# zzyunzhi/object-intrinsics

Hardware: AMD Instinct MI355X
Metric: rendered rays/sec (64x64 img, 128 samples/ray) + D-images/sec (higher is better)
Workload: dtype f32 via f16x3 (fp32 operands split into 2 fp16 limbs = 22 mantissa bits, 3 fp16 MFMAs per product, fp32 accumulate: 2^-22 relative per product, 1e-4 parity path); 1 GPU; C2: 1x64x64 crop per GPU, 64+64 samples/ray, 1 up-sampling step(s), Generator.forward (render + Phong maps) + ADADiscriminatorView forward; parallelism=dp1 (independent renders, no data-path collective)

## Files before the change

### object-intrinsics_amd/build.py

```python
import hashlib
import os
import subprocess
import sys

HERE = os.path.dirname(os.path.abspath(__file__))
CSRC = os.path.join(HERE, "csrc")
OUT_DIR = os.path.join(HERE, "oi_amd")
LIB = os.path.join(OUT_DIR, "liboi_hip.so")
STAMP = os.path.join(OUT_DIR, ".liboi_hip.stamp")
SOURCES = ["mlp.hip", "mlp_fwd3.hip", "mlp_fwd3b.hip", "color_head.hip", "render.hip", "disc.hip", "disc_small.hip", "disc_large.hip", "mlp_bwd.hip", "render_bwd.hip", "disc_bwd.hip", "optim.hip", "loss.hip", "mesh.hip", "relight.hip"]
FLAGS = ["--offload-arch=gfx950", "-O3", "-std=c++17", "-fPIC", "-Wno-unused-value"] + os.environ.get("OI_FLAGS", "").split()
EXTRA = {"mlp_fwd3.hip": ["-mllvm", "-amdgpu-mfma-vgpr-form=1"],
         "mlp_fwd3b.hip": ["-mllvm", "-amdgpu-mfma-vgpr-form=1", "-fno-slp-vectorize"],
         "mlp_bwd.hip": ["-mllvm", "-amdgpu-mfma-vgpr-form=1"]}


def _hipcc():
    for c in (os.environ.get("HIPCC"), "/opt/rocm/bin/hipcc", "hipcc"):
        if c and (os.path.isabs(c) and os.path.exists(c) or not os.path.isabs(c)):
            return c
    raise RuntimeError("hipcc not found")


def _sources():
    return [s for s in SOURCES if os.path.exists(os.path.join(CSRC, s))]


def _digest():
    h = hashlib.sha256()
    files = [os.path.join(CSRC, f) for f in sorted(os.listdir(CSRC))]
    inc = os.path.join(os.path.dirname(HERE), "include")
    files += [os.path.join(inc, f) for f in sorted(os.listdir(inc))]
    for f in files:
        with open(f, "rb") as fh:
            h.update(os.path.basename(f).encode())
            h.update(fh.read())
    h.update(" ".join(FLAGS).encode())
    h.update(repr(EXTRA).encode())
    return h.hexdigest()


def build(force=False, verbose=True):
    dig = _digest()
    if not force and os.path.exists(LIB) and os.path.exists(STAMP) and open(STAMP).read() == dig:
        return LIB
    hipcc = _hipcc()
    objs = []
    procs = []
    os.makedirs(os.path.join(HERE, "build"), exist_ok=True)
    for s in _sources():
        o = os.path.join(HERE, "build", s.replace(".hip", ".o"))
        cmd = [hipcc, *FLAGS, *EXTRA.get(s, []), "-c", os.path.join(CSRC, s), "-o", o]
        if verbose:
            print(" ".join(cmd), flush=True)
        procs.append((s, subprocess.Popen(cmd, stdout=subprocess.PIPE, stderr=subprocess.STDOUT)))
        objs.append(o)
    for s, p in procs:
        out, _ = p.communicate()
        if p.returncode != 0:
            raise RuntimeError(f"hipcc failed on {s}:\n{out.decode()}")
    cmd = [hipcc, "--offload-arch=gfx950", "-shared", "-fPIC", "-o", LIB, *objs]
    if verbose:
        print(" ".join(cmd), flush=True)
    subprocess.check_call(cmd)
    with open(STAMP, "w") as fh:
        fh.write(dig)
    return LIB


if __name__ == "__main__":
    print(build(force="--force" in sys.argv))
```

### object-intrinsics_amd/csrc/mlp.hip

```cpp
#include <cstdlib>

#include <algorithm>

#include "mlp_common.h"
#include "f3_blob.h"

namespace {

using namespace oimlp;

__global__ void film_params_kernel(const float* __restrict__ style_w, const float* __restrict__ style_b,
                                   const float* __restrict__ z, float* __restrict__ w_out,
                                   const float* __restrict__ gw, const float* __restrict__ gb,
                                   const float* __restrict__ bw, const float* __restrict__ bb,
                                   float* __restrict__ gamma, float* __restrict__ beta, int NL) {
  __shared__ float h[2][64];
  const int e = blockIdx.x, t = threadIdx.x;
  if (z != nullptr) {
    if (t < 64) h[0][t] = z[e * 64 + t];
    __syncthreads();
    int cur = 0;
    for (int l = 0; l < 3; ++l) {
      if (t < 64) {
        const float* wr = style_w + (l * 64 + t) * 64;
// ... 119 lines not shown
    __syncthreads();
    for (int o = part; o < 64; o += 4) atomicAdd(d_style_w + (l * 64 + o) * 64 + t, dh[cur][o] * h[l][t]);
    if (tid < 64) {
      float acc = 0.f;
#pragma unroll 8
      for (int o = 0; o < 64; ++o) acc = fmaf(dh[cur][o], W[l][o][t], acc);
      dh[cur ^ 1][t] = acc;
    }
    __syncthreads();
    cur ^= 1;
  }
  if (d_z != nullptr && tid < 64) d_z[e * 64 + t] = dh[cur][t];
}

__device__ __forceinline__ float mat_elem(const float* wh, const float* wv, int m, int row, int k) {
  if (m < 7) return wh[((size_t)m * C + row) * C + k];
  if (m < 14) return wh[((size_t)(m - 7) * C + k) * C + row];
  if (m == 14) return wv[(size_t)row * (C + 3) + k];
  return wv[(size_t)k * (C + 3) + row];
}

template <int PREC>
__device__ float image_scale(const float* wh, const float* wv, int m, float* red, float* inv, float* bad,
                             float* rowsum = nullptr) {
  *bad = 0.f;
  if (PREC != OI_PREC_F16X3) {
    *inv = 1.f;
    return 1.f;
  }
  float mx = 0.f;
  for (int i = threadIdx.x; i < C * C; i += 256) {
    const float a = fabsf(mat_elem(wh, wv, m, i >> 7, i & 127));
    mx = a <= 3.0e38f ? fmaxf(mx, a) : __builtin_inff();
    if (rowsum != nullptr) atomicAdd(rowsum + (i >> 7), a);
  }
  red[threadIdx.x] = mx;
  __syncthreads();
  for (int o = 128; o > 0; o >>= 1) {
    if ((int)threadIdx.x < o) red[threadIdx.x] = fmaxf(red[threadIdx.x], red[threadIdx.x + o]);
    __syncthreads();
  }
  mx = red[0];
  __syncthreads();
  *bad = mx <= 3.0e38f ? 0.f : 1.f;
  int eb = (__builtin_bit_cast(int, mx) >> 23) & 0xff;
  eb = eb < 14 ? 14 : (eb > 254 ? 254 : eb);
  *inv = __builtin_bit_cast(float, (eb - 13) << 23);
  return __builtin_bit_cast(float, (267 - eb) << 23);
}

constexpr int PK_PER = 8;

template <int PREC>
__global__ void pack_weights_kernel(const float* __restrict__ w0, const float* __restrict__ b0,
                                    const float* __restrict__ wh, const float* __restrict__ bh,
                                    const float* __restrict__ wsig, const float* __restrict__ bsig,
                                    const float* __restrict__ wv, const float* __restrict__ bv,
                                    const float* __restrict__ wrgb, const float* __restrict__ brgb,
                                    char* __restrict__ packed) {
  float* hdr = reinterpret_cast<float*>(packed);
  __shared__ float red[256];
  if (blockIdx.y == NMAT) {
   for (int idx = blockIdx.x * blockDim.x + threadIdx.x; idx < H_FLOATS; idx += gridDim.x * blockDim.x) {
    if ((idx >= H_WSCALE && idx < H_WSCALE + NMAT) || (idx >= H_BOUND && idx < H_BOUND + NMAT) ||
        (idx >= H_STATUS && idx < H_STATUS + NMAT))
      continue;
    float v = 0.f;
    if (idx < H_SIG) {
      int f = idx >> 2, j = idx & 3;
      v = j < 3 ? w0[f * 3 + j] : 0.f;
    } else if (idx < H_TABV) {
      int i = idx - H_SIG;
      v = i < C ? wsig[i] : (i == C ? bsig[0] : 0.f);
    } else if (idx < H_RGB) {
      int i = idx - H_TABV, f = i >> 2, j = i & 3;
      v = j < 3 ? wv[(size_t)f * (C + 3) + C + j] : 0.f;
    } else if (idx < H_TABS_END) {
      int i = idx - H_RGB;
      v = i < 3 * C ? wrgb[i] : (i < 3 * C + 3 ? brgb[i - 3 * C] : 0.f);
    } else if (idx < H_BIAS + 9 * C) {
      int i = idx - H_BIAS, l = i / C, f = i % C;
      v = l == 0 ? b0[f] : (l < 8 ? bh[(l - 1) * C + f] : bv[f]);
    }
    hdr[idx] = v;
   }
    return;
  }
  const int m = blockIdx.y;
  float inv, bad;
  __shared__ float rowsum[C];
  if (threadIdx.x < C) rowsum[threadIdx.x] = 0.f;
  __syncthreads();
  const float wscale = image_scale<PREC>(wh, wv, m, red, &inv, &bad, blockIdx.x == 0 ? rowsum : nullptr);
  if (blockIdx.x == 0 && threadIdx.x == 0) {
    hdr[H_WSCALE + m] = inv;
    hdr[H_STATUS + m] = bad;
  }
  if (blockIdx.x == 0) {
    float rs = 0.f;
    if (threadIdx.x < C) {
      if (PREC == OI_PREC_F16X3) rs = rowsum[threadIdx.x];
      else for (int k = 0; k < C; ++k) rs += fabsf(mat_elem(wh, wv, m, threadIdx.x, k));
    }
    red[threadIdx.x] = rs;
    __syncthreads();
    for (int o = 128; o > 0; o >>= 1) {
      if ((int)threadIdx.x < o) red[threadIdx.x] = fmaxf(red[threadIdx.x], red[threadIdx.x + o]);
      __syncthreads();
    }
    if (threadIdx.x == 0) hdr[H_BOUND + m] = red[0] * wscale;
    __syncthreads();
  }
  for (int part = 0; part < PK_PER; ++part) {
  const int idx = (blockIdx.x * PK_PER + part) * blockDim.x + threadIdx.x;
  if (idx >= C * C) return;
  if (m < 7 || m == 14)
    reinterpret_cast<float*>(packed + plain_off(PREC))[(size_t)(m < 7 ? m : 7) * C * C + idx] =
        mat_elem(wh, wv, m, idx >> 7, idx & 127);
  char* base = packed + H_BYTES + (size_t)m * layer_bytes(PREC);
  if (PREC == OI_PREC_F32) {
    const int k = idx & 3, lane = (idx >> 2) & 63, g = (idx >> 8) & 15, t = idx >> 12;
    const int q = 4 * g + k, h = lane >> 5, i = lane & 31;
    reinterpret_cast<float*>(base)[idx] = mat_elem(wh, wv, m, 32 * t + i, feat_of(q, h));
  } else {
    const int ip = idx & 7, lane = (idx >> 3) & 63, s = (idx >> 9) & 7, t = idx >> 12;
    const int q = 8 * s + ip, h = lane >> 5, i = lane & 31;
    const float v = mat_elem(wh, wv, m, 32 * t + i, feat_of(q, h)) * wscale;
    if (PREC == OI_PREC_F16X3) {
      const _Float16 fh = (_Float16)v;
      reinterpret_cast<_Float16*>(base)[idx] = fh;
      reinterpret_cast<_Float16*>(base + 32768)[idx] = (_Float16)(v - (float)fh);
      continue;
    }
    const __bf16 hi = (__bf16)v;
    reinterpret_cast<__bf16*>(base)[idx] = hi;
    if (PREC == OI_PREC_BF16X3) reinterpret_cast<__bf16*>(base + 32768)[idx] = (__bf16)(v - (float)hi);
    if (PREC == OI_PREC_BF16X6) {
      const float r1 = v - (float)hi;
      const __bf16 mid = (__bf16)r1;
      reinterpret_cast<__bf16*>(base + 32768)[idx] = mid;
      reinterpret_cast<__bf16*>(base + 65536)[idx] = (__bf16)(r1 - (float)mid);
    }
  }
  }
}


template <bool FAST>
__device__ __forceinline__ float sin_rev(float phi_rev) {
  return __builtin_amdgcn_sinf(FAST ? phi_rev : __builtin_amdgcn_fractf(phi_rev));
}
template <bool FAST, bool FULL, int SRC, class SCR, bool REV = false>
__device__ __forceinline__ void film_sin2(const char* lds, const LaneOff& o, const LayOff& y, const f32x16 (&acc)[4],
                                          float (&act)[64], const SCR& ws, int slot, int tab_imm, float vx,
                                          float vy, float vz) {
#pragma unroll
  for (int g = 0; g < 16; ++g) {
    const int t = g >> 2, rr = g & 3;
    const f32x4 gm = lds_f4(lds, grp_f0(g) * 4, y.f16);
    const f32x4 bt = lds_f4(lds, (C + grp_f0(g)) * 4, y.f16);
    f32x4 cv;
#pragma unroll
    for (int k = 0; k < 4; ++k) {
      float u;
      if constexpr (SRC == 0) {
        u = acc[t][4 * rr + k];
      } else {
        const f32x4 w = lds_f4(lds, V2_TABS + tab_imm * 4 + (grp_f0(g) + k) * 16, o.h64);
        const float d = fmaf(vz, w[2], fmaf(vy, w[1], vx * w[0]));
        u = SRC == 1 ? d : acc[t][4 * rr + k] + d;
      }
      const float phi = fmaf(gm[k], u, bt[k]);
      if constexpr (REV) {
        act[4 * g + k] = sin_rev<FAST>(phi);
      } else {
        float s, c;
        sincos_<FAST>(phi, s, c);
        act[4 * g + k] = s;
        cv[k] = gm[k] * c;
      }
    }
    if constexpr (FULL) ws.store(slot, g, o, cv);
    if ((g & 1) == 1) __builtin_amdgcn_sched_barrier(0);
  }
}

template <bool FAST, bool FULL, bool REV, class SCR>
__device__ __forceinline__ void layer_fwd_pipelined(const char* lds, const LaneOff& o, const LayOff& y,
                                                    f32x16 (&acc)[4], float (&act)[64], const SCR& ws, int slot) {
  f16x8 bh[8], bl[8];
#pragma unroll
  for (int s = 0; s < 8; ++s) split8_pairs(&act[8 * s], bh[s], bl[s]);
  f32x4 gm, bt, cv;
  auto film_val = [&](int tb, int s, int j) {
    const int g = tb * 4 + (s >> 1), k = 2 * (s & 1) + j;
    if (k == 0) {
      gm = lds_f4(lds, grp_f0(g) * 4, y.f16);
      bt = lds_f4(lds, (C + grp_f0(g)) * 4, y.f16);
    }
    const float phi = fmaf(gm[k], acc[tb][2 * s + j], bt[k]);
    if constexpr (REV) {
      act[4 * g + k] = sin_rev<FAST>(phi);
    } else {
      float sn, cs;
      sincos_<FAST>(phi, sn, cs);
      act[4 * g + k] = sn;
      cv[k] = gm[k] * cs;
    }
    if constexpr (FULL) {
      if (k == 3) ws.store(slot, g, o, cv);
    }
  };
  auto film_part = [&](int tb, int s) {
    film_val(tb, s, 0);
    film_val(tb, s, 1);
  };
  f32x4 ah = lds_f4(lds, 0, y.wl), al = lds_f4(lds, 0, y.wh), ahn = ah, aln = al;
#pragma unroll
  for (int t = 0; t < 4; ++t) {
#pragma unroll
    for (int r = 0; r < 16; ++r) acc[t][r] = 0.f;
#pragma unroll
    for (int s = 0; s < 8; ++s) {
      const int nxt = t * 8 + s + 1;
      if (nxt < 32) {
        ahn = lds_f4(lds, nxt * 1024, y.wl);
        aln = lds_f4(lds, nxt * 1024, y.wh);
      }
      const f16x8 wh = __builtin_bit_cast(f16x8, ah);
      const f16x8 wl = __builtin_bit_cast(f16x8, al);
      acc[t] = __builtin_amdgcn_mfma_f32_32x32x16_f16(wl, bh[s], acc[t], 0, 0, 0);
      if (t > 0) {
        film_val(t - 1, s, 0);
        __builtin_amdgcn_sched_barrier(0);
      }
      acc[t] = __builtin_amdgcn_mfma_f32_32x32x16_f16(wh, bl[s], acc[t], 0, 0, 0);
      if (t > 0) {
        film_val(t - 1, s, 1);
        __builtin_amdgcn_sched_barrier(0);
      }
      acc[t] = __builtin_amdgcn_mfma_f32_32x32x16_f16(wh, bh[s], acc[t], 0, 0, 0);
      __builtin_amdgcn_sched_barrier(0);
      ah = ahn;
      al = aln;
    }
  }
#pragma unroll
  for (int s = 0; s < 8; ++s) {
    film_part(3, s);
    if (s & 1) __builtin_amdgcn_sched_barrier(0);
  }
}

__device__ __forceinline__ void zero_acc(f32x16 (&acc)[4]) {
#pragma unroll
  for (int t = 0; t < 4; ++t)
#pragma unroll
    for (int r = 0; r < 16; ++r) acc[t][r] = 0.f;
}

#ifdef OI_PROF
__device__ unsigned long long oi_prof[16];
#define PROF_T(i)                                                  \
  do {                                                             \
    const unsigned long long t_ = __builtin_readcyclecounter();    \
    pacc[i] += t_ - tprev;                                         \
    tprev = t_;                                                    \
  } while (0)
#else
#define PROF_T(i)
#endif

#define OI_SDF_LATTICE 0
#include "sdf_mlp_kernel.inc"
#undef OI_SDF_LATTICE

#define OI_LATTICE_POINT(x, y, z)                                                                            \
  do {                                                                                                       \
    const unsigned loc_ = (unsigned)(pt - (long long)e * n_per_elem), nyz_ = (unsigned)lat_ny * lat_nz;      \
    const unsigned ix_ = loc_ / nyz_, r_ = loc_ - ix_ * nyz_, iy_ = r_ / (unsigned)lat_nz;                   \
    x = xs[ix_], y = ys[iy_], z = zs[r_ - iy_ * (unsigned)lat_nz];                                           \
  } while (0)
#define OI_SDF_LATTICE 1
#include "sdf_mlp_kernel.inc"
#undef OI_SDF_LATTICE
#undef OI_LATTICE_POINT

template <int PREC, bool FAST, bool FULL>
int launch_mlp_variant(const float* pts, const char* pk, const float* gamma, const float* beta, float* sdf, float* grad,
                       float* rgb, float* feat, char* scratch, int B, long long n, hipStream_t st) {
  constexpr int NWV = V2_WAVES;
  constexpr int LDS_BYTES = v2_lds_total(PREC);
  static const int per_dev = [] {
    const char* v = getenv("OI_V2_PERSIST");
    if (v && v[0] == '0') return 0;
    int dev = 0, cus = 256;
    (void)hipGetDevice(&dev);
    (void)hipDeviceGetAttribute(&cus, hipDeviceAttributeMultiprocessorCount, dev);
    return cus > 0 ? cus : 256;
  }();
  const int tiles = oi::cdiv(n, NWV * WAVE_PTS);
  const bool persist = !FULL && v2_two_slots(PREC) && per_dev > 0;
  dim3 grid(persist ? std::min(tiles, std::max(1, per_dev / B)) : tiles, B), block(64 * NWV);
  auto k = sdf_mlp_kernel<PREC, FAST, FULL>;
  (void)hipFuncSetAttribute(reinterpret_cast<const void*>(k), hipFuncAttributeMaxDynamicSharedMemorySize, LDS_BYTES);
  hipLaunchKernelGGL(k, grid, block, LDS_BYTES, st, pts, pk, gamma, beta, sdf, grad, rgb, feat, scratch, n);
  return oi::check_launch("oi_sdf_mlp_fwd");
}

template <int PREC, bool FAST>
int launch_lattice(const float* xs, const float* ys, const float* zs, int ny, int nz, float scale, const char* pk,
                   const float* gamma, const float* beta, float* out, int B, long long n, hipStream_t st) {
  constexpr int NWV = V2_WAVES;
  constexpr int LDS_BYTES = v2_lds_total(PREC);
  static const int cus = [] {
    int dev = 0, c = 256;
    (void)hipGetDevice(&dev);
    (void)hipDeviceGetAttribute(&c, hipDeviceAttributeMultiprocessorCount, dev);
    return c > 0 ? c : 256;
  }();
  const int tiles = oi::cdiv(n, NWV * WAVE_PTS);
  dim3 grid(v2_two_slots(PREC) ? std::min(tiles, std::max(1, cus / B)) : tiles, B), block(64 * NWV);
  auto k = sdf_lattice_kernel<PREC, FAST, false>;
  static std::atomic<unsigned long long> set{0};
  int dev = 0;
  (void)hipGetDevice(&dev);
  if (dev >= 64 || !((set.load() >> dev) & 1ull)) {
    if (hipFuncSetAttribute(reinterpret_cast<const void*>(k), hipFuncAttributeMaxDynamicSharedMemorySize, LDS_BYTES) !=
        hipSuccess)
      return oi::fail(OI_ERR_LAUNCH, "oi_sdf_lattice: hipFuncSetAttribute(%d B of LDS) failed", LDS_BYTES);
    if (dev < 64) set.fetch_or(1ull << dev);
  }
  hipLaunchKernelGGL(k, grid, block, LDS_BYTES, st, xs, ys, zs, ny, nz, scale, pk, gamma, beta, out, n);
  return oi::check_launch("oi_sdf_lattice");
}

template <int PREC, bool FAST>
int launch_mlp(const float* pts, const void* packed, const float* gamma, const float* beta, float* sdf,
               float* grad, float* rgb, float* feat, void* scratch, int B, long long n, hipStream_t st) {
  const char* pk = reinterpret_cast<const char*>(packed);
  if (grad != nullptr) {
    if constexpr (PREC == OI_PREC_F16X3 || PREC == OI_PREC_BF16)
      return oi::fail(OI_ERR_INVALID_ARG, "oi_sdf_mlp_fwd: precision %d with the gradient has no v2 kernel", PREC);
    else
      return launch_mlp_variant<PREC, FAST, true>(pts, pk, gamma, beta, sdf, grad, rgb, feat,
                                                  reinterpret_cast<char*>(scratch), B, n, st);
  }
  return launch_mlp_variant<PREC, FAST, false>(pts, pk, gamma, beta, sdf, nullptr, nullptr, feat, nullptr, B, n, st);
}

template <bool FAST>
__global__ void selftest_sincos_kernel(const float* __restrict__ x, float* __restrict__ s, float* __restrict__ c,
                                       long long n) {
  const long long i = (long long)blockIdx.x * blockDim.x + threadIdx.x;
  if (i >= n) return;
  float sv, cv;
  sincos_<FAST>(x[i], sv, cv);
  s[i] = sv;
  c[i] = cv;
}

}

extern "C" {

int oi_film_params(const float* style_w, const float* style_b, const float* z, float* w_out, const float* gw,
                   const float* gb, const float* bw, const float* bb, float* gamma, float* beta, int B, int NL,
                   oi_stream_t stream) {
  OI_REQUIRE(B > 0 && NL >= 0, "oi_film_params: B=%d NL=%d", B, NL);
  OI_REQUIRE(w_out && (NL == 0 || (gw && gb && bw && bb && gamma && beta)), "oi_film_params: null pointer");
  OI_REQUIRE(z == nullptr || (style_w && style_b), "oi_film_params: z given without style weights");
  hipLaunchKernelGGL(film_params_kernel, dim3(B, NL > 0 ? NL : 1), dim3(C), 0, oi::as_stream(stream), style_w, style_b, z, w_out,
                     gw, gb, bw, bb, gamma, beta, NL);
  return oi::check_launch("oi_film_params");
}

#ifdef OI_PROF
int oi_prof_read(unsigned long long* out, int reset) {
  (void)hipDeviceSynchronize();
  (void)hipMemcpyFromSymbol(out, HIP_SYMBOL(oi_prof), sizeof(unsigned long long) * 16);
  if (reset) {
    unsigned long long z[16] = {0};
    (void)hipMemcpyToSymbol(HIP_SYMBOL(oi_prof), z, sizeof(z));
  }
  return 0;
}
#endif

int oi_film_params_bwd(const float* d_gamma, const float* d_beta, const float* w, const float* gw, const float* bw,
                       float* d_gw, float* d_gb, float* d_bw, float* d_bb, float* d_w, const float* style_w,
                       const float* style_b, const float* z, float* d_style_w, float* d_style_b, float* d_z, int B,
                       int NL, oi_stream_t stream) {
  OI_REQUIRE(B > 0 && NL >= 0 && (NL > 0 || z != nullptr), "oi_film_params_bwd: B=%d NL=%d", B, NL);
  OI_REQUIRE(d_w && (NL == 0 || (d_gamma && d_beta && w && gw && bw && d_gw && d_gb && d_bw && d_bb)),
             "oi_film_params_bwd: null pointer");
  OI_REQUIRE(z == nullptr || (style_w && style_b && d_style_w && d_style_b),
             "oi_film_params_bwd: style backward needs style_w, style_b, d_style_w, d_style_b");
  hipStream_t st = oi::as_stream(stream);
  int rc = OI_OK;
  if (NL > 0) {
    hipLaunchKernelGGL(film_heads_bwd_kernel, dim3(NL), dim3(256), 0, st, d_gamma, d_beta, w, gw, bw, d_gw, d_gb, d_bw,
                       d_bb, d_w, B, NL);
    rc = oi::check_launch("oi_film_params_bwd(heads)");
  }
  if (rc != OI_OK || z == nullptr) return rc;
  hipLaunchKernelGGL(style_bwd_kernel, dim3(B), dim3(256), 0, st, style_w, style_b, z, d_w, d_style_w, d_style_b, d_z);
  return oi::check_launch("oi_film_params_bwd(style)");
}

size_t oi_mlp_packed_bytes(int prec) { return packed_total_bytes(prec); }

int oi_mlp_pack_weights(const float* w0, const float* b0, const float* wh, const float* bh, const float* wsig,
                        const float* bsig, const float* wv, const float* bv, const float* wrgb, const float* brgb,
                        void* packed, int prec, oi_stream_t stream) {
  OI_REQUIRE(w0 && b0 && wh && bh && wsig && bsig && wv && bv && wrgb && brgb && packed,
             "oi_mlp_pack_weights: null pointer");
  dim3 grid(C * C / (256 * PK_PER), NMAT + 1), block(256);
  char* p = reinterpret_cast<char*>(packed);
  hipStream_t st = oi::as_stream(stream);
  switch (prec) {
    case OI_PREC_F32:
      hipLaunchKernelGGL(pack_weights_kernel<OI_PREC_F32>, grid, block, 0, st, w0, b0, wh, bh, wsig, bsig, wv, bv,
                         wrgb, brgb, p);
      break;
    case OI_PREC_BF16X3:
      hipLaunchKernelGGL(pack_weights_kernel<OI_PREC_BF16X3>, grid, block, 0, st, w0, b0, wh, bh, wsig, bsig, wv, bv,
                         wrgb, brgb, p);
      break;
    case OI_PREC_BF16:
      hipLaunchKernelGGL(pack_weights_kernel<OI_PREC_BF16>, grid, block, 0, st, w0, b0, wh, bh, wsig, bsig, wv, bv,
                         wrgb, brgb, p);
      break;
    case OI_PREC_BF16X6:
      hipLaunchKernelGGL(pack_weights_kernel<OI_PREC_BF16X6>, grid, block, 0, st, w0, b0, wh, bh, wsig, bsig, wv, bv,
                         wrgb, brgb, p);
      break;
    case OI_PREC_F16X3:
      hipLaunchKernelGGL(pack_weights_kernel<OI_PREC_F16X3>, grid, block, 0, st, w0, b0, wh, bh, wsig, bsig, wv, bv,
                         wrgb, brgb, p);
      break;
    default:
      return oi::fail(OI_ERR_INVALID_ARG, "oi_mlp_pack_weights: bad precision %d", prec);
  }
  return oi::check_launch("oi_mlp_pack_weights");
}

int oi_selftest_sincos(const float* x, float* s, float* c, long long n, int fast, oi_stream_t stream) {
  OI_REQUIRE(x && s && c && n > 0, "oi_selftest_sincos: bad argument");
  if (fast)
    hipLaunchKernelGGL(selftest_sincos_kernel<true>, dim3(oi::cdiv(n, 256)), dim3(256), 0, oi::as_stream(stream), x, s, c, n);
  else
    hipLaunchKernelGGL(selftest_sincos_kernel<false>, dim3(oi::cdiv(n, 256)), dim3(256), 0, oi::as_stream(stream), x, s, c, n);
  return oi::check_launch("oi_selftest_sincos");
}

int oi_mlp_pack_status(const void* packed, oi_stream_t stream) {
  OI_REQUIRE(packed, "oi_mlp_pack_status: null pointer");
  hipStream_t st = oi::as_stream(stream);
  static thread_local float host[H_FLOATS];
  if (hipMemcpyAsync(host, packed, sizeof(host), hipMemcpyDeviceToHost, st) != hipSuccess || hipStreamSynchronize(st) != hipSuccess)
    return oi::fail(OI_ERR_LAUNCH, "oi_mlp_pack_status: reading the packed header failed");
  for (int m = 0; m < NMAT; ++m)
    if (host[H_STATUS + m] != 0.f)
      return oi::fail(OI_ERR_UNSUPPORTED, "oi_mlp_pack_status: weight image %d holds a non-finite value (inf / NaN)", m);
  for (int i = 0; i < H_BIAS + 9 * C; ++i)
    if (!(host[i] >= -3.0e38f && host[i] <= 3.0e38f))
      return oi::fail(OI_ERR_UNSUPPORTED, "oi_mlp_pack_status: non-finite first-layer / head weight or bias (header float %d)", i);
  return OI_OK;
}

size_t oi_mlp_scratch_bytes(int B, long long n_per_elem) {
  const long long tiles = (n_per_elem + V2_TILE - 1) / V2_TILE;
  return (size_t)B * tiles * V2_WAVES * NSLOT * 16 * 64 * 16;
}

size_t oi_mlp_scratch_bytes_prec(int B, long long n_per_elem, int prec) {
  if (prec == OI_PREC_F16X3) return oimlp::full3_scratch_bytes(B, n_per_elem);
  if (prec == OI_PREC_BF16) return oimlp::full3_bf16_scratch_bytes(B);
  return oi_mlp_scratch_bytes(B, n_per_elem);
}

int oi_sdf_mlp_fwd(const float* pts, const void* packed, const float* gamma, const float* beta, float* sdf,
                   float* grad, float* rgb, float* feat, void* scratch, int B, long long n_per_elem, int prec,
                   int fast_trig, oi_stream_t stream) {
  return oi_sdf_mlp_fwd_ex(pts, packed, gamma, beta, sdf, grad, rgb, feat, scratch, B, n_per_elem, prec, fast_trig, 0, stream);
}

size_t oi_mlp_f3_blob_offset(int B, long long n_per_elem) { return oimlp::full3_blob_offset(B, n_per_elem); }
size_t oi_mlp_f3_blob_bytes(void) { return (size_t)oif3::F3_BLOB; }

int oi_sdf_mlp_fwd_ex(const float* pts, const void* packed, const float* gamma, const float* beta, float* sdf,
                      float* grad, float* rgb, float* feat, void* scratch, int B, long long n_per_elem, int prec,
                      int fast_trig, int flags, oi_stream_t stream) {
  OI_REQUIRE(pts && packed && gamma && beta && sdf, "oi_sdf_mlp_fwd: null pointer");
  OI_REQUIRE((flags & ~OI_MLP_BLOB_READY) == 0, "oi_sdf_mlp_fwd_ex: unknown flag bits %d", flags);
  OI_REQUIRE(!(flags & OI_MLP_BLOB_READY) || (prec == OI_PREC_F16X3 && grad != nullptr),
             "oi_sdf_mlp_fwd_ex: OI_MLP_BLOB_READY applies to the OI_PREC_F16X3 pass with the gradient");
  OI_REQUIRE(B > 0 && n_per_elem > 0, "oi_sdf_mlp_fwd: B=%d n=%lld", B, n_per_elem);
  OI_REQUIRE(grad != nullptr || rgb == nullptr, "oi_sdf_mlp_fwd: rgb requires grad");
  OI_REQUIRE(grad == nullptr || scratch != nullptr, "oi_sdf_mlp_fwd: grad requires scratch");
  hipStream_t st = oi::as_stream(stream);
  if (prec == OI_PREC_F16X3 && grad != nullptr)
    return oimlp::launch_full3_f16x3(pts, packed, gamma, beta, sdf, grad, rgb, feat, scratch, B, n_per_elem, fast_trig,
                                     (flags & OI_MLP_BLOB_READY) != 0, st);
  if (prec == OI_PREC_BF16 && grad != nullptr)
    return oimlp::launch_full3_bf16(pts, packed, gamma, beta, sdf, grad, rgb, feat, scratch, B, n_per_elem, fast_trig, st);
#define OI_MLP_CASE(P)                                                                                        \
  case P:                                                                                                     \
    return fast_trig ? launch_mlp<P, true>(pts, packed, gamma, beta, sdf, grad, rgb, feat, scratch, B, n_per_elem, st) \
                     : launch_mlp<P, false>(pts, packed, gamma, beta, sdf, grad, rgb, feat, scratch, B, n_per_elem, st);
  switch (prec) {
    OI_MLP_CASE(OI_PREC_F32)
    OI_MLP_CASE(OI_PREC_BF16X3)
    OI_MLP_CASE(OI_PREC_BF16)
    OI_MLP_CASE(OI_PREC_BF16X6)
    OI_MLP_CASE(OI_PREC_F16X3)
    default:
      return oi::fail(OI_ERR_INVALID_ARG, "oi_sdf_mlp_fwd: bad precision %d", prec);
  }
#undef OI_MLP_CASE
}

int oi_sdf_lattice(const void* packed, const float* gamma, const float* beta, int B, const float* xs, const float* ys,
                   const float* zs, int nx, int ny, int nz, float scale, float* out, int prec, int fast_trig,
                   oi_stream_t stream) {
  OI_REQUIRE(packed && gamma && beta && xs && ys && zs && out, "oi_sdf_lattice: null pointer");
  OI_REQUIRE(B > 0 && nx > 0 && ny > 0 && nz > 0, "oi_sdf_lattice: B=%d nx=%d ny=%d nz=%d", B, nx, ny, nz);
  const long long n = (long long)nx * ny * nz;
  OI_REQUIRE(n < (1ll << 31), "oi_sdf_lattice: %d x %d x %d = %lld points per element (at most 2^31 - 1)", nx, ny, nz, n);
  const char* pk = reinterpret_cast<const char*>(packed);
  hipStream_t st = oi::as_stream(stream);
#define OI_LAT_CASE(P)                                                                                           \
  case P:                                                                                                        \
    return fast_trig ? launch_lattice<P, true>(xs, ys, zs, ny, nz, scale, pk, gamma, beta, out, B, n, st)        \
                     : launch_lattice<P, false>(xs, ys, zs, ny, nz, scale, pk, gamma, beta, out, B, n, st);
  switch (prec) {
    OI_LAT_CASE(OI_PREC_F32)
    OI_LAT_CASE(OI_PREC_BF16X3)
    OI_LAT_CASE(OI_PREC_BF16)
    OI_LAT_CASE(OI_PREC_BF16X6)
    OI_LAT_CASE(OI_PREC_F16X3)
    default:
      return oi::fail(OI_ERR_INVALID_ARG, "oi_sdf_lattice: bad precision %d", prec);
  }
#undef OI_LAT_CASE
}

}
```

### object-intrinsics_amd/csrc/mlp_common.h

```cpp
#pragma once
#include "oi_common.h"

namespace oimlp {

typedef float f32x16 __attribute__((ext_vector_type(16)));
typedef float f32x4 __attribute__((ext_vector_type(4)));
typedef __bf16 bf16x8 __attribute__((ext_vector_type(8)));
typedef _Float16 f16x8 __attribute__((ext_vector_type(8)));

constexpr int C = 128;
constexpr int NL_SDF = 8;
constexpr int NMAT = 16;
constexpr int TILE_PTS = 128;
constexpr int WAVE_PTS = 32;
constexpr int NSLOT = 9;

constexpr int H_TAB0 = 0;
constexpr int H_SIG = 512;
constexpr int H_TABV = 656;
constexpr int H_RGB = 1168;
constexpr int H_TABS_END = 1568;
constexpr int H_BIAS = 1568;
constexpr int H_WSCALE = 2720;
constexpr int H_BOUND = 2736;
// ... 123 lines not shown
        for (int t = 0; t < 4; ++t)
          acc[t] = __builtin_amdgcn_mfma_f32_32x32x2f32(a[t][k], act[4 * g + k], acc[t], 0, 0, 0);
      }
      if (g & 1) hook(g >> 1);
      __builtin_amdgcn_sched_barrier(0);
#pragma unroll
      for (int t = 0; t < 4; ++t) a[t] = an[t];
    }
  } else if constexpr (PREC == OI_PREC_BF16X6) {
#pragma unroll
    for (int s = 0; s < 8; ++s) {
      bf16x8 bh, bm, bl;
#pragma unroll
      for (int i = 0; i < 8; ++i) {
        const float v = act[8 * s + i];
        bh[i] = (__bf16)v;
        const float r1 = v - (float)bh[i];
        bm[i] = (__bf16)r1;
        bl[i] = (__bf16)(r1 - (float)bm[i]);
      }
#pragma unroll
      for (int t = 0; t < 4; ++t) {
        const bf16x8 wh = __builtin_bit_cast(bf16x8, lds_f4(lds, (t * 8 + s) * 1024, y.wl));
        const bf16x8 wm = __builtin_bit_cast(bf16x8, lds_f4(lds, (t * 8 + s) * 1024, y.wh));
        const bf16x8 wl = __builtin_bit_cast(bf16x8, lds_f4(lds, (t * 8 + s) * 1024, y.wq));
        acc[t] = __builtin_amdgcn_mfma_f32_32x32x16_bf16(wl, bh, acc[t], 0, 0, 0);
        acc[t] = __builtin_amdgcn_mfma_f32_32x32x16_bf16(wh, bl, acc[t], 0, 0, 0);
        acc[t] = __builtin_amdgcn_mfma_f32_32x32x16_bf16(wm, bm, acc[t], 0, 0, 0);
        acc[t] = __builtin_amdgcn_mfma_f32_32x32x16_bf16(wm, bh, acc[t], 0, 0, 0);
        acc[t] = __builtin_amdgcn_mfma_f32_32x32x16_bf16(wh, bm, acc[t], 0, 0, 0);
        acc[t] = __builtin_amdgcn_mfma_f32_32x32x16_bf16(wh, bh, acc[t], 0, 0, 0);
      }
      hook(s);
      __builtin_amdgcn_sched_barrier(0);
    }
  } else if constexpr (PREC == OI_PREC_F16X3) {
    f32x4 ah[4], ahn[4], al[4], aln[4];
#pragma unroll
    for (int t = 0; t < 4; ++t) {
      ah[t] = lds_f4(lds, (t * 8 + 0) * 1024, y.wl);
      al[t] = lds_f4(lds, (t * 8 + 0) * 1024, y.wh);
    }
#pragma unroll
    for (int s = 0; s < 8; ++s) {
      if (s < 7) {
#pragma unroll
        for (int t = 0; t < 4; ++t) {
          ahn[t] = lds_f4(lds, (t * 8 + s + 1) * 1024, y.wl);
          aln[t] = lds_f4(lds, (t * 8 + s + 1) * 1024, y.wh);
        }
      }
      f16x8 bh, bl;
      split8_pairs(&act[8 * s], bh, bl);
#pragma unroll
      for (int t = 0; t < 4; ++t) {
        const f16x8 wh = __builtin_bit_cast(f16x8, ah[t]);
        const f16x8 wl = __builtin_bit_cast(f16x8, al[t]);
        acc[t] = __builtin_amdgcn_mfma_f32_32x32x16_f16(wl, bh, acc[t], 0, 0, 0);
        acc[t] = __builtin_amdgcn_mfma_f32_32x32x16_f16(wh, bl, acc[t], 0, 0, 0);
        acc[t] = __builtin_amdgcn_mfma_f32_32x32x16_f16(wh, bh, acc[t], 0, 0, 0);
      }
      hook(s);
      __builtin_amdgcn_sched_barrier(0);
#pragma unroll
      for (int t = 0; t < 4; ++t) {
        ah[t] = ahn[t];
        al[t] = aln[t];
      }
    }
  } else {
    f32x4 ah[4], ahn[4], al[4], aln[4];
#pragma unroll
    for (int t = 0; t < 4; ++t) {
      ah[t] = lds_f4(lds, (t * 8 + 0) * 1024, y.wl);
      if constexpr (PREC == OI_PREC_BF16X3) al[t] = lds_f4(lds, (t * 8 + 0) * 1024, y.wh);
    }
#pragma unroll
    for (int s = 0; s < 8; ++s) {
      if (s < 7) {
#pragma unroll
        for (int t = 0; t < 4; ++t) {
          ahn[t] = lds_f4(lds, (t * 8 + s + 1) * 1024, y.wl);
          if constexpr (PREC == OI_PREC_BF16X3) aln[t] = lds_f4(lds, (t * 8 + s + 1) * 1024, y.wh);
        }
      }
      bf16x8 bh, bl;
#pragma unroll
      for (int i = 0; i < 8; ++i) {
        const float v = act[8 * s + i];
        bh[i] = (__bf16)v;
        if constexpr (PREC == OI_PREC_BF16X3) bl[i] = (__bf16)(v - (float)bh[i]);
      }
#pragma unroll
      for (int t = 0; t < 4; ++t) {
        const bf16x8 wh = __builtin_bit_cast(bf16x8, ah[t]);
        if constexpr (PREC == OI_PREC_BF16X3) {
          const bf16x8 wl = __builtin_bit_cast(bf16x8, al[t]);
          acc[t] = __builtin_amdgcn_mfma_f32_32x32x16_bf16(wl, bh, acc[t], 0, 0, 0);
          acc[t] = __builtin_amdgcn_mfma_f32_32x32x16_bf16(wh, bl, acc[t], 0, 0, 0);
        }
        acc[t] = __builtin_amdgcn_mfma_f32_32x32x16_bf16(wh, bh, acc[t], 0, 0, 0);
      }
      hook(s);
      __builtin_amdgcn_sched_barrier(0);
#pragma unroll
      for (int t = 0; t < 4; ++t) {
        ah[t] = ahn[t];
        if constexpr (PREC == OI_PREC_BF16X3) al[t] = aln[t];
      }
    }
  }
}

template <int PREC>
__device__ __forceinline__ void gemm_layer(const char* lds, const LaneOff& o, const float (&act)[64],
                                           f32x16 (&acc)[4]) {
  LayOff y;
  y.wl = o.l16 + L_WBUF;
  y.wh = o.l16hi + L_WBUF;
  y.wq = y.wl + 65536;
  y.f16 = 0;
  gemm_layer2<PREC>(lds, y, act, acc);
}

template <bool FAST>
__device__ __forceinline__ void sincos_(float x, float& s, float& c) {
  if constexpr (FAST) {
    s = __sinf(x);
    c = __cosf(x);
  } else {
    const float q = x * 0.15915494309189533577f;
    const float n = __builtin_rintf(q);
    float r = fmaf(x, 0.15915494309189533577f, -n);
    r = fmaf(x, 6.4206383266e-09f, r);
    s = __builtin_amdgcn_sinf(r);
    c = __builtin_amdgcn_cosf(r);
  }
}

struct WaveScratch {
  __amdgpu_buffer_rsrc_t rs;
  __device__ __forceinline__ void store(int slot, int g, int l16, f32x4 v) const {
    oi::buffer_store_b128<oi::FWD_NT_ST>(__builtin_bit_cast(u32x4, v), rs, l16, slot * 16384 + g * 1024);
  }
  __device__ __forceinline__ f32x4 load(int slot, int g, int l16) const {
    return __builtin_bit_cast(f32x4, __builtin_amdgcn_raw_buffer_load_b128(rs, l16, slot * 16384 + g * 1024, oi::FWD_NT_LD));
  }
};

template <bool FAST, bool FULL, int SRC>
__device__ __forceinline__ void film_sin(const char* lds, const LaneOff& o, const f32x16 (&acc)[4],
                                         float (&act)[64], const WaveScratch& ws, int slot, int tab_imm,
                                         float vx, float vy, float vz) {
#pragma unroll
  for (int g = 0; g < 16; ++g) {
    const int t = g >> 2, rr = g & 3;
    const f32x4 gm = lds_f4(lds, L_FILM + grp_f0(g) * 4, o.h16);
    const f32x4 bt = lds_f4(lds, L_FILM + (C + grp_f0(g)) * 4, o.h16);
    f32x4 bs;
    if constexpr (SRC == 1) bs = lds_f4(lds, L_FILM + (2 * C + grp_f0(g)) * 4, o.h16);
    f32x4 cv;
#pragma unroll
    for (int k = 0; k < 4; ++k) {
      float u;
      if constexpr (SRC == 0) {
        u = acc[t][4 * rr + k];
      } else {
        const f32x4 w = lds_f4(lds, L_TABS + tab_imm * 4 + (grp_f0(g) + k) * 16, o.h64);
        const float d = fmaf(vz, w[2], fmaf(vy, w[1], vx * w[0]));
        u = SRC == 1 ? d + bs[k] : acc[t][4 * rr + k] + d;
      }
      const float phi = fmaf(gm[k], u, bt[k]);
      float s, c;
      sincos_<FAST>(phi, s, c);
      act[4 * g + k] = s;
      cv[k] = gm[k] * c;
    }
    if constexpr (FULL) ws.store(slot, g, o.l16, cv);
    __builtin_amdgcn_sched_barrier(0);
  }
}

__device__ __forceinline__ float pow2_normalise(float (&act)[64], float* lane_max = nullptr) {
  float m = 0.f;
#pragma unroll
  for (int k = 0; k < 64; k += 2) m = fmaxf(m, fmaxf(fabsf(act[k]), fabsf(act[k + 1])));
  if (lane_max != nullptr) *lane_max = m;
  m = fmaxf(m, __shfl_xor(m, 32, 64));
  int eb = (__builtin_bit_cast(int, m) >> 23) & 0xff;
  eb = eb < 14 ? 14 : (eb > 254 ? 254 : eb);
  float sc = __builtin_bit_cast(float, (267 - eb) << 23);
  asm volatile("" : "+v"(sc) : : "memory");
#pragma unroll
  for (int k = 0; k < 64; ++k) act[k] *= sc;
  return __builtin_bit_cast(float, (eb - 13) << 23);
}

template <int PREC, bool NORM>
__device__ __forceinline__ float gemm_scaled(const char* lds, const LaneOff& o, float (&act)[64], f32x16 (&acc)[4],
                                             float inv_img) {
  float f = 1.f;
  if constexpr (PREC == OI_PREC_F16X3) {
    f = inv_img;
    if constexpr (NORM) f *= pow2_normalise(act);
  }
  gemm_layer<PREC>(lds, o, act, acc);
  return f;
}

__device__ __forceinline__ void acc_zero(f32x16 (&acc)[4]) {
#pragma unroll
  for (int t = 0; t < 4; ++t)
#pragma unroll
    for (int r = 0; r < 16; ++r) acc[t][r] = 0.f;
}

__device__ __forceinline__ void init_bias(const char* lds, const LaneOff& o, f32x16 (&acc)[4]) {
#pragma unroll
  for (int g = 0; g < 16; ++g) {
    const f32x4 b = lds_f4(lds, L_FILM + (2 * C + grp_f0(g)) * 4, o.h16);
#pragma unroll
    for (int k = 0; k < 4; ++k) acc[g >> 2][4 * (g & 3) + k] = b[k];
  }
}


typedef _Float16 f16x4 __attribute__((ext_vector_type(4)));
typedef unsigned int u32x2 __attribute__((ext_vector_type(2)));
template <bool HALF>
struct FwdScratch {
  __amdgpu_buffer_rsrc_t rs;
  __device__ __forceinline__ void store(int slot, int g, const LaneOff& o, f32x4 v) const {
    if constexpr (HALF) {
      f16x4 hv;
#pragma unroll
      for (int k = 0; k < 4; ++k) hv[k] = (_Float16)v[k];
      __builtin_amdgcn_raw_buffer_store_b64(__builtin_bit_cast(u32x2, hv), rs, o.l16 >> 1, slot * 8192 + g * 512, 0);
    } else {
      oi::buffer_store_b128<oi::FWD_NT_ST>(__builtin_bit_cast(u32x4, v), rs, o.l16, slot * 16384 + g * 1024);
    }
  }
  __device__ __forceinline__ f32x4 load(int slot, int g, const LaneOff& o) const {
    if constexpr (HALF) {
      const f16x4 hv = __builtin_bit_cast(f16x4, __builtin_amdgcn_raw_buffer_load_b64(rs, o.l16 >> 1, slot * 8192 + g * 512, 0));
      f32x4 v;
#pragma unroll
      for (int k = 0; k < 4; ++k) v[k] = (float)hv[k];
      return v;
    } else {
      return __builtin_bit_cast(f32x4, __builtin_amdgcn_raw_buffer_load_b128(rs, o.l16, slot * 16384 + g * 1024, oi::FWD_NT_LD));
    }
  }
};

constexpr int V2_WAVES = 8;
constexpr int V2_TILE = V2_WAVES * WAVE_PTS;
constexpr int V2_FILM = 0;
constexpr int V2_TABS = 9 * 1024;
constexpr int V2_WBUF = V2_TABS + H_TABS_END * 4;
__host__ __device__ constexpr bool v2_two_slots(int prec) { return prec != OI_PREC_BF16X6; }
__host__ __device__ constexpr int v2_lds_total(int prec) {
  return V2_WBUF + (v2_two_slots(prec) ? 2 : 1) * layer_bytes(prec);
}


template <int PREC, int NWAVES>
__device__ __forceinline__ void prefetch_image(char* lds, __amdgpu_buffer_rsrc_t rs, int src_off, int slot, int wave, int l16) {
  constexpr int PER_WAVE = layer_bytes(PREC) / NWAVES;
  static_assert(PER_WAVE % 4096 == 0, "a wave's share of an image is a multiple of 4 KiB");
#pragma unroll
  for (int q = 0; q < PER_WAVE / 4096; ++q) {
    const int c = wave * PER_WAVE + q * 4096;
    auto* dst = (__attribute__((address_space(3))) void*)(lds + V2_WBUF + slot * layer_bytes(PREC) + c);
    __builtin_amdgcn_raw_ptr_buffer_load_lds(rs, dst, 16, l16, src_off + c, 0, 0);
    __builtin_amdgcn_raw_ptr_buffer_load_lds(rs, dst, 16, l16, src_off + c, 1024, 0);
    __builtin_amdgcn_raw_ptr_buffer_load_lds(rs, dst, 16, l16, src_off + c, 2048, 0);
    __builtin_amdgcn_raw_ptr_buffer_load_lds(rs, dst, 16, l16, src_off + c, 3072, 0);
  }
}

template <int PREC>
__device__ __forceinline__ LayOff lay_off(const LaneOff& o, int slot, int layer) {
  LayOff r;
  r.wl = o.l16 + V2_WBUF + slot * layer_bytes(PREC);
  r.wh = r.wl + 32768;
  r.wq = r.wl + 65536;
  r.f16 = o.h16 + V2_FILM + layer * 1024;
  return r;
}

template <int TRAILING = 0>
__device__ __forceinline__ void ring_sync() {
  asm volatile("s_waitcnt vmcnt(%0)" ::"n"(TRAILING) : "memory");
  __syncthreads();
}


size_t full3_scratch_bytes(int B, long long n_per_elem);
size_t full3_blob_offset(int B, long long n_per_elem);
int launch_full3_f16x3(const float* pts, const void* packed, const float* gamma, const float* beta, float* sdf,
                       float* grad, float* rgb, float* feat, void* scratch, int B, long long n, int fast_trig, bool blob_ready,
                       hipStream_t st);

size_t full3_bf16_scratch_bytes(int B);
int launch_full3_bf16(const float* pts, const void* packed, const float* gamma, const float* beta, float* sdf, float* grad,
                      float* rgb, float* feat, void* scratch, int B, long long n, int fast_trig, hipStream_t st);

}
```

Before: 3.649 million rays/s.

## Add two-point-per-lane SDF-only f16x3 MLP kernel with interleaved sine epilogue

Adds a specialized persistent kernel for the SDF-only forward path (no features) in which each wave processes two 32-point groups, P and Q, sharing each LDS weight fragment load. The SIREN sine and limb-split epilogue of the previous layer is interleaved with the current layer's MFMAs using sched_group_barrier hints, and the output head is folded into the last layer's epilogue. The aim is to hide transcendental and VALU work behind the MFMAs and to halve weight-load traffic per point. The cost is much higher register pressure, which is why the kernel is pinned to one wave per EU. It is enabled by default and can be turned off with OI_SDF2=0.

```diff
diff --git a/object-intrinsics_amd/build.py b/object-intrinsics_amd/build.py
--- a/object-intrinsics_amd/build.py
+++ b/object-intrinsics_amd/build.py
@@ -8,9 +8,10 @@
 OUT_DIR = os.path.join(HERE, "oi_amd")
 LIB = os.path.join(OUT_DIR, "liboi_hip.so")
 STAMP = os.path.join(OUT_DIR, ".liboi_hip.stamp")
-SOURCES = ["mlp.hip", "mlp_fwd3.hip", "mlp_fwd3b.hip", "color_head.hip", "render.hip", "disc.hip", "disc_small.hip", "disc_large.hip", "mlp_bwd.hip", "render_bwd.hip", "disc_bwd.hip", "optim.hip", "loss.hip", "mesh.hip", "relight.hip"]
+SOURCES = ["mlp.hip", "mlp_sdf2.hip", "mlp_fwd3.hip", "mlp_fwd3b.hip", "color_head.hip", "render.hip", "disc.hip", "disc_small.hip", "disc_large.hip", "mlp_bwd.hip", "render_bwd.hip", "disc_bwd.hip", "optim.hip", "loss.hip", "mesh.hip", "relight.hip"]
 FLAGS = ["--offload-arch=gfx950", "-O3", "-std=c++17", "-fPIC", "-Wno-unused-value"] + os.environ.get("OI_FLAGS", "").split()
 EXTRA = {"mlp_fwd3.hip": ["-mllvm", "-amdgpu-mfma-vgpr-form=1"],
+         "mlp_sdf2.hip": ["-mllvm", "-amdgpu-mfma-vgpr-form=1"],
          "mlp_fwd3b.hip": ["-mllvm", "-amdgpu-mfma-vgpr-form=1", "-fno-slp-vectorize"],
          "mlp_bwd.hip": ["-mllvm", "-amdgpu-mfma-vgpr-form=1"]}
 
diff --git a/object-intrinsics_amd/csrc/mlp.hip b/object-intrinsics_amd/csrc/mlp.hip
--- a/object-intrinsics_amd/csrc/mlp.hip
+++ b/object-intrinsics_amd/csrc/mlp.hip
@@ -445,6 +445,13 @@
   const int tiles = oi::cdiv(n, NWV * WAVE_PTS);
   const bool persist = !FULL && v2_two_slots(PREC) && per_dev > 0;
   dim3 grid(persist ? std::min(tiles, std::max(1, per_dev / B)) : tiles, B), block(64 * NWV);
+  if constexpr (PREC == OI_PREC_F16X3 && !FULL) {
+    static const bool sdf2 = [] {
+      const char* v = getenv("OI_SDF2");
+      return !(v && v[0] == '0');
+    }();
+    if (sdf2 && feat == nullptr) return launch_sdf2_f16x3(pts, pk, gamma, beta, sdf, grid, n, FAST, st);
+  }
   auto k = sdf_mlp_kernel<PREC, FAST, FULL>;
   (void)hipFuncSetAttribute(reinterpret_cast<const void*>(k), hipFuncAttributeMaxDynamicSharedMemorySize, LDS_BYTES);
   hipLaunchKernelGGL(k, grid, block, LDS_BYTES, st, pts, pk, gamma, beta, sdf, grad, rgb, feat, scratch, n);
diff --git a/object-intrinsics_amd/csrc/mlp_common.h b/object-intrinsics_amd/csrc/mlp_common.h
--- a/object-intrinsics_amd/csrc/mlp_common.h
+++ b/object-intrinsics_amd/csrc/mlp_common.h
@@ -449,6 +449,9 @@
                        float* grad, float* rgb, float* feat, void* scratch, int B, long long n, int fast_trig, bool blob_ready,
                        hipStream_t st);
 
+int launch_sdf2_f16x3(const float* pts, const char* pk, const float* gamma, const float* beta, float* sdf, dim3 grid,
+                      long long n, bool fast_trig, hipStream_t st);
+
 size_t full3_bf16_scratch_bytes(int B);
 int launch_full3_bf16(const float* pts, const void* packed, const float* gamma, const float* beta, float* sdf, float* grad,
                       float* rgb, float* feat, void* scratch, int B, long long n, int fast_trig, hipStream_t st);
diff --git a/object-intrinsics_amd/csrc/mlp_sdf2.hip b/object-intrinsics_amd/csrc/mlp_sdf2.hip
--- /dev/null
+++ b/object-intrinsics_amd/csrc/mlp_sdf2.hip
@@ -0,0 +1,309 @@
+#include <type_traits>
+
+#include "mlp_common.h"
+
+namespace {
+
+using namespace oimlp;
+
+constexpr int S2_WAVES = 4;
+constexpr int S2_TILE = S2_WAVES * 2 * WAVE_PTS;
+static_assert(S2_TILE == V2_TILE, "launch_mlp_variant sizes the grid for both kernels");
+constexpr int S2_PREC = OI_PREC_F16X3;
+constexpr int S2_LB = layer_bytes(S2_PREC);
+constexpr int S2_LDS = v2_lds_total(S2_PREC);
+
+typedef unsigned Limbs[8][4];
+
+struct NoTail2 {
+  __device__ __forceinline__ void operator()(int, int) const {}
+};
+template <class T> struct is_no_tail2 { static constexpr bool value = false; };
+template <> struct is_no_tail2<NoTail2> { static constexpr bool value = true; };
+
+__device__ __forceinline__ f16x8 limb_frag(const Limbs& b, int s) {
+  const u32x4 u = {b[s][0], b[s][1], b[s][2], b[s][3]};
+  return __builtin_bit_cast(f16x8, u);
+}
+
+constexpr int S2_VALU_PER_MFMA = 2;
+constexpr int S2_TRANS_PER_MFMA = 1;
+
+template <class TAIL, class EPI>
+__device__ __forceinline__ void stream_layer2(const char* lds, const LayOff& y, const Limbs& ph, const Limbs& pl,
+                                              const Limbs& qh, const Limbs& ql, f32x16 (&accP)[4], f32x16 (&accQ)[4],
+                                              TAIL&& tail, EPI&& epi) {
+  constexpr bool HAS_TAIL = !is_no_tail2<std::remove_cv_t<std::remove_reference_t<TAIL>>>::value;
+  f32x4 ah[2], al[2];
+  ah[0] = lds_f4(lds, 0, y.wl);
+  al[0] = lds_f4(lds, 0, y.wh);
+#pragma unroll
+  for (int t = 0; t < 4; ++t) {
+#pragma unroll
+    for (int r = 0; r < 16; ++r) {
+      accP[t][r] = 0.f;
+      accQ[t][r] = 0.f;
+    }
+#pragma unroll
+    for (int s = 0; s < 8; ++s) {
+      const int cur = t * 8 + s, nxt = cur + 1;
+      if (nxt < 32) {
+        ah[nxt & 1] = lds_f4(lds, nxt * 1024, y.wl);
+        al[nxt & 1] = lds_f4(lds, nxt * 1024, y.wh);
+      }
+      int npairs = 0;
+      if (t == 0) {
+        if (HAS_TAIL && s < 6) {
+          constexpr int first[7] = {0, 2, 3, 4, 6, 7, 8};
+          for (int rp = first[s]; rp < first[s + 1]; ++rp) tail(3, rp);
+          npairs = first[s + 1] - first[s];
+        }
+      } else {
+        epi(t - 1, s);
+        npairs = 1;
+      }
+      const f16x8 wh = __builtin_bit_cast(f16x8, ah[cur & 1]);
+      const f16x8 wl = __builtin_bit_cast(f16x8, al[cur & 1]);
+      const f16x8 vhP = limb_frag(ph, s), vlP = limb_frag(pl, s), vhQ = limb_frag(qh, s), vlQ = limb_frag(ql, s);
+      accP[t] = __builtin_amdgcn_mfma_f32_32x32x16_f16(wl, vhP, accP[t], 0, 0, 0);
+      accQ[t] = __builtin_amdgcn_mfma_f32_32x32x16_f16(wl, vhQ, accQ[t], 0, 0, 0);
+      accP[t] = __builtin_amdgcn_mfma_f32_32x32x16_f16(wh, vlP, accP[t], 0, 0, 0);
+      accQ[t] = __builtin_amdgcn_mfma_f32_32x32x16_f16(wh, vlQ, accQ[t], 0, 0, 0);
+      accP[t] = __builtin_amdgcn_mfma_f32_32x32x16_f16(wh, vhP, accP[t], 0, 0, 0);
+      accQ[t] = __builtin_amdgcn_mfma_f32_32x32x16_f16(wh, vhQ, accQ[t], 0, 0, 0);
+      if (npairs >= 1) {
+#pragma unroll
+        for (int q = 0; q < 5; ++q) {
+          __builtin_amdgcn_sched_group_barrier(0x008, 1, 0);
+          if (npairs <= 1) {
+            __builtin_amdgcn_sched_group_barrier(0x002, S2_VALU_PER_MFMA, 0);
+            __builtin_amdgcn_sched_group_barrier(0x400, S2_TRANS_PER_MFMA, 0);
+          } else {
+            __builtin_amdgcn_sched_group_barrier(0x002, 2 * S2_VALU_PER_MFMA, 0);
+            __builtin_amdgcn_sched_group_barrier(0x400, 2 * S2_TRANS_PER_MFMA, 0);
+          }
+        }
+        __builtin_amdgcn_sched_group_barrier(0x008, 1, 0);
+      }
+      __builtin_amdgcn_sched_barrier(0);
+    }
+  }
+}
+template <class EPI>
+__device__ __forceinline__ void run_tail2(EPI&& epi) {
+#pragma unroll
+  for (int rp = 0; rp < 8; ++rp) {
+    epi(3, rp);
+    if (rp & 1) __builtin_amdgcn_sched_barrier(0);
+  }
+}
+
+template <bool FAST>
+__global__ void __launch_bounds__(64 * S2_WAVES) __attribute__((amdgpu_waves_per_eu(1, 1)))
+sdf_mlp_sdf2_kernel(const float* __restrict__ pts, const char* __restrict__ packed, const float* __restrict__ gamma,
+                    const float* __restrict__ beta, float* __restrict__ sdf_out, long long n_per_elem) {
+  extern __shared__ __attribute__((aligned(16))) char lds[];
+  const int tid = threadIdx.x, lane = tid & 63;
+  const int wave = __builtin_amdgcn_readfirstlane(tid >> 6);
+  const int h = lane >> 5, j = lane & 31;
+  const int e = blockIdx.y;
+  const float* hdr = reinterpret_cast<const float*>(packed);
+  const char* mats = packed + H_BYTES;
+  constexpr int NT = 64 * S2_WAVES;
+
+  LaneOff o;
+  o.h16 = 16 * h;
+  o.h64 = 64 * h;
+  o.l16 = 16 * lane;
+  o.l16hi = 16 * lane + 32768;
+  asm volatile("" : "+v"(o.h16), "+v"(o.h64), "+v"(o.l16), "+v"(o.l16hi));
+
+  const __amdgpu_buffer_rsrc_t img_rs =
+      __builtin_amdgcn_make_buffer_rsrc(const_cast<char*>(mats), 0, NMAT * S2_LB, 0x00020000);
+  auto stage = [&](int image, int slot) { prefetch_image<S2_PREC, S2_WAVES>(lds, img_rs, image * S2_LB, slot, wave, o.l16); };
+
+  const int ntiles = (int)((n_per_elem + S2_TILE - 1) / S2_TILE);
+  int tile = blockIdx.x, rb = 0;
+  auto point_of = [&](int t_, int q, bool& valid) {
+    const long long local = (long long)t_ * S2_TILE + wave * (2 * WAVE_PTS) + q * WAVE_PTS + j;
+    valid = local < n_per_elem;
+    return (long long)e * n_per_elem + (valid ? local : n_per_elem - 1);
+  };
+
+  stage(0, 0);
+  {
+    float* tabs = reinterpret_cast<float*>(lds + V2_TABS);
+    for (int i = tid; i < H_TABS_END; i += NT) tabs[i] = hdr[i];
+    float* film = reinterpret_cast<float*>(lds + V2_FILM);
+    for (int i = tid; i < 9 * C; i += NT) {
+      const int l = i / C, f = i % C;
+      const float gm = gamma[((size_t)e * 9 + l) * C + f];
+      const float ws = l == 0 ? 1.f : hdr[H_WSCALE + (l < NL_SDF ? l - 1 : 14)];
+      constexpr float TO_REV = 0.15915494309189533577f;
+      film[l * 256 + f] = gm * ws * TO_REV;
+      film[l * 256 + C + f] = fmaf(gm, hdr[H_BIAS + l * C + f], beta[((size_t)e * 9 + l) * C + f]) * TO_REV;
+    }
+  }
+  float pxP, pyP, pzP, pxQ, pyQ, pzQ;
+  {
+    bool v;
+    const long long a = point_of(tile, 0, v), b = point_of(tile, 1, v);
+    pxP = pts[a * 3 + 0], pyP = pts[a * 3 + 1], pzP = pts[a * 3 + 2];
+    pxQ = pts[b * 3 + 0], pyQ = pts[b * 3 + 1], pzQ = pts[b * 3 + 2];
+  }
+  __syncthreads();
+
+  f32x16 accP[4], accQ[4];
+  Limbs AHP, ALP, AHQ, ALQ, BHP, BLP, BHQ, BLQ;
+  struct Rows {
+    f32x4 a, b, d;
+  } rw[2];
+
+  auto reduce = [&](float phi) { return FAST ? phi : __builtin_amdgcn_fractf(phi); };
+  auto film_base = [&](int l) { return o.h16 + V2_FILM + l * 1024; };
+#define ROW_A(FB, G) lds_f4(lds, grp_f0(G) * 4, FB)
+#define ROW_B(FB, G) lds_f4(lds, (C + grp_f0(G)) * 4, FB)
+#define ROW_SIG(G) lds_f4(lds, V2_TABS + (H_SIG + grp_f0(G)) * 4, o.h16)
+#define NEXT_AB(FB) (rw[0].a = ROW_A(FB, 0), rw[0].b = ROW_B(FB, 0))
+
+#define OI_S2_EPI(FB, NHP, NLP, NHQ, NLQ, NEXT)                                                                 \
+  [&](int tb, int rp) {                                                                                         \
+    const int g = tb * 4 + (rp >> 1), k = 2 * (rp & 1);                                                         \
+    Rows& R = rw[g & 1];                                                                                        \
+    if (k == 0) {                                                                                               \
+      if (g < 15) {                                                                                             \
+        rw[(g + 1) & 1].a = ROW_A(FB, g + 1);                                                                   \
+        rw[(g + 1) & 1].b = ROW_B(FB, g + 1);                                                                   \
+      } else {                                                                                                  \
+        NEXT;                                                                                                   \
+      }                                                                                                         \
+    }                                                                                                           \
+    const float p0 = reduce(fmaf(R.a[k], accP[tb][2 * rp], R.b[k]));                                            \
+    const float p1 = reduce(fmaf(R.a[k + 1], accP[tb][2 * rp + 1], R.b[k + 1]));                                \
+    const float q0 = reduce(fmaf(R.a[k], accQ[tb][2 * rp], R.b[k]));                                            \
+    const float q1 = reduce(fmaf(R.a[k + 1], accQ[tb][2 * rp + 1], R.b[k + 1]));                                \
+    split_pair(__builtin_amdgcn_sinf(p0), __builtin_amdgcn_sinf(p1), NHP[2 * tb + (rp >> 2)][rp & 3],           \
+               NLP[2 * tb + (rp >> 2)][rp & 3]);                                                                \
+    split_pair(__builtin_amdgcn_sinf(q0), __builtin_amdgcn_sinf(q1), NHQ[2 * tb + (rp >> 2)][rp & 3],           \
+               NLQ[2 * tb + (rp >> 2)][rp & 3]);                                                                \
+  }
+
+  const int F0 = film_base(0), F1 = film_base(1), F2 = film_base(2), F3 = film_base(3), F4 = film_base(4),
+            F5 = film_base(5), F6 = film_base(6), F7 = film_base(7);
+  float sdfP = 0.f, sdfQ = 0.f;
+  auto e1 = OI_S2_EPI(F1, BHP, BLP, BHQ, BLQ, NEXT_AB(F2));
+  auto e2 = OI_S2_EPI(F2, AHP, ALP, AHQ, ALQ, NEXT_AB(F3));
+  auto e3 = OI_S2_EPI(F3, BHP, BLP, BHQ, BLQ, NEXT_AB(F4));
+  auto e4 = OI_S2_EPI(F4, AHP, ALP, AHQ, ALQ, NEXT_AB(F5));
+  auto e5 = OI_S2_EPI(F5, BHP, BLP, BHQ, BLQ, NEXT_AB(F6));
+  auto e6 = OI_S2_EPI(F6, AHP, ALP, AHQ, ALQ, (NEXT_AB(F7), rw[0].d = ROW_SIG(0)));
+  auto e7 = [&](int tb, int rp) {
+    const int g = tb * 4 + (rp >> 1), k = 2 * (rp & 1);
+    Rows& R = rw[g & 1];
+    if (k == 0 && g < 15) {
+      Rows& N = rw[(g + 1) & 1];
+      N.a = ROW_A(F7, g + 1);
+      N.b = ROW_B(F7, g + 1);
+      N.d = ROW_SIG(g + 1);
+    }
+#pragma unroll
+    for (int i = 0; i < 2; ++i) {
+      const float sp = __builtin_amdgcn_sinf(reduce(fmaf(R.a[k + i], accP[tb][2 * rp + i], R.b[k + i])));
+      const float sq = __builtin_amdgcn_sinf(reduce(fmaf(R.a[k + i], accQ[tb][2 * rp + i], R.b[k + i])));
+      sdfP = fmaf(sp, R.d[k + i], sdfP);
+      sdfQ = fmaf(sq, R.d[k + i], sdfQ);
+    }
+  };
+
+  for (;;) {
+    const int ntile = tile + (int)gridDim.x;
+    const bool more = ntile < ntiles;
+    float nxP, nyP, nzP, nxQ, nyQ, nzQ;
+    {
+      bool v;
+      const long long a = point_of(more ? ntile : tile, 0, v), b = point_of(more ? ntile : tile, 1, v);
+      nxP = pts[a * 3 + 0], nyP = pts[a * 3 + 1], nzP = pts[a * 3 + 2];
+      nxQ = pts[b * 3 + 0], nyQ = pts[b * 3 + 1], nzQ = pts[b * 3 + 2];
+    }
+
+#pragma unroll
+    for (int g = 0; g < 16; ++g) {
+      const f32x4 gm = ROW_A(F0, g), bt = ROW_B(F0, g);
+      float sp[4], sq[4];
+#pragma unroll
+      for (int k = 0; k < 4; ++k) {
+        const f32x4 w = lds_f4(lds, V2_TABS + H_TAB0 * 4 + (grp_f0(g) + k) * 16, o.h64);
+        const float uP = fmaf(pzP, w[2], fmaf(pyP, w[1], pxP * w[0]));
+        const float uQ = fmaf(pzQ, w[2], fmaf(pyQ, w[1], pxQ * w[0]));
+        sp[k] = __builtin_amdgcn_sinf(reduce(fmaf(gm[k], uP, bt[k])));
+        sq[k] = __builtin_amdgcn_sinf(reduce(fmaf(gm[k], uQ, bt[k])));
+      }
+      split_pair(sp[0], sp[1], AHP[g >> 1][2 * (g & 1)], ALP[g >> 1][2 * (g & 1)]);
+      split_pair(sp[2], sp[3], AHP[g >> 1][2 * (g & 1) + 1], ALP[g >> 1][2 * (g & 1) + 1]);
+      split_pair(sq[0], sq[1], AHQ[g >> 1][2 * (g & 1)], ALQ[g >> 1][2 * (g & 1)]);
+      split_pair(sq[2], sq[3], AHQ[g >> 1][2 * (g & 1) + 1], ALQ[g >> 1][2 * (g & 1) + 1]);
+      __builtin_amdgcn_sched_barrier(0);
+    }
+    NEXT_AB(F1);
+    ring_sync();
+
+    stage(1, 1 ^ rb);
+    stream_layer2(lds, lay_off<S2_PREC>(o, 0 ^ rb, 1), AHP, ALP, AHQ, ALQ, accP, accQ, NoTail2(), e1);
+    ring_sync();
+    stage(2, 0 ^ rb);
+    stream_layer2(lds, lay_off<S2_PREC>(o, 1 ^ rb, 2), BHP, BLP, BHQ, BLQ, accP, accQ, e1, e2);
+    ring_sync();
+    stage(3, 1 ^ rb);
+    stream_layer2(lds, lay_off<S2_PREC>(o, 0 ^ rb, 3), AHP, ALP, AHQ, ALQ, accP, accQ, e2, e3);
+    ring_sync();
+    stage(4, 0 ^ rb);
+    stream_layer2(lds, lay_off<S2_PREC>(o, 1 ^ rb, 4), BHP, BLP, BHQ, BLQ, accP, accQ, e3, e4);
+    ring_sync();
+    stage(5, 1 ^ rb);
+    stream_layer2(lds, lay_off<S2_PREC>(o, 0 ^ rb, 5), AHP, ALP, AHQ, ALQ, accP, accQ, e4, e5);
+    ring_sync();
+    stage(6, 0 ^ rb);
+    stream_layer2(lds, lay_off<S2_PREC>(o, 1 ^ rb, 6), BHP, BLP, BHQ, BLQ, accP, accQ, e5, e6);
+    ring_sync();
+    if (more) stage(0, 1 ^ rb);
+    sdfP = 0.f, sdfQ = 0.f;
+    stream_layer2(lds, lay_off<S2_PREC>(o, 0 ^ rb, 7), AHP, ALP, AHQ, ALQ, accP, accQ, e6, e7);
+    run_tail2(e7);
+
+    {
+      sdfP += __shfl_xor(sdfP, 32, 64);
+      sdfQ += __shfl_xor(sdfQ, 32, 64);
+      const float bsig = *reinterpret_cast<const float*>(lds + V2_TABS + (H_SIG + C) * 4);
+      bool vP, vQ;
+      const long long a = point_of(tile, 0, vP), b = point_of(tile, 1, vQ);
+      if (vP && h == 0) sdf_out[a] = sdfP + bsig;
+      if (vQ && h == 0) sdf_out[b] = sdfQ + bsig;
+    }
+
+    if (!more) break;
+    tile = ntile;
+    rb ^= 1;
+    pxP = nxP, pyP = nyP, pzP = nzP;
+    pxQ = nxQ, pyQ = nyQ, pzQ = nzQ;
+  }
+#undef OI_S2_EPI
+#undef NEXT_AB
+#undef ROW_A
+#undef ROW_B
+#undef ROW_SIG
+}
+
+}
+
+namespace oimlp {
+
+int launch_sdf2_f16x3(const float* pts, const char* pk, const float* gamma, const float* beta, float* sdf, dim3 grid,
+                      long long n, bool fast_trig, hipStream_t st) {
+  const dim3 block(64 * S2_WAVES);
+  auto k = fast_trig ? sdf_mlp_sdf2_kernel<true> : sdf_mlp_sdf2_kernel<false>;
+  (void)hipFuncSetAttribute(reinterpret_cast<const void*>(k), hipFuncAttributeMaxDynamicSharedMemorySize, S2_LDS);
+  hipLaunchKernelGGL(k, grid, block, S2_LDS, st, pts, pk, gamma, beta, sdf, n);
+  return oi::check_launch("oi_sdf_mlp_fwd(sdf2)");
+}
+
+}
```

Measured after the change: 3.658 million rays/s (median of 6 runs). Within noise of the previous version (+0.3%).
